# driskai/scenario_gym

Hardware: AMD Instinct MI355X
Metric: entity-steps/sec (batched rollout) (higher is better)
Workload: dtype f64

## Files before the change

scenario_gym_amd/csrc/h_queue.hip:

```cpp
#include "sgym_host.hpp"

using namespace sgh;

enum { Q_HOST_RING = 16 };
int sgh::check_queue(sg_handle *h)
{
    for (; h->q_count > 0; --h->q_count) {
        const unsigned *w = h->q_host + (size_t)((h->q_head - h->q_count + Q_HOST_RING) % Q_HOST_RING) * sg::Q_STATE_WORDS;
        const unsigned code = w[sg::Q_ERR];
        if (code == 0 || h->q_failed) continue;
        static const char *what[] = {"", "a rollout wavefront waited for the controller pre-pass", "a rollout wavefront waited for the previous chunk of its block",
                                     "the controller pre-pass waited for a buffer of the table ring"};
        h->q_failed = true;
        h->queue_mode = 0;
        snprintf(h->q_msg, sizeof h->q_msg, "sg_rollout: the persistent table launch gave up (%s longer than SG_QUEUE_TIMEOUT_MS; %u work items had finished): "
                                            "the state of the batch is undefined -- sg_reset / sg_upload before the next call", what[code < 4 ? code : 0],
                 w[sg::Q_ITEMS_DONE]);
    }
    return h->q_failed ? fail(h, SG_ERR_HIP, "%s", h->q_msg) : SG_OK;
}
void sgh::forget_queue_failure(sg_handle *h)
{
    h->q_count = 0;
    h->q_failed = false;
}

#define SG_QUEUE_FALLBACK 1
static size_t slots_of(sg_handle *h, bool rss)
{
    const size_t by_bounds = (size_t)h->n_simd * (size_t)(rss ? SG_WAVES_PER_SIMD : (h->planar ? SG_PLANAR_WAVES : SG_TAB_WAVES));
    if (h->q_waves_G != h->G) {
        std::fill(h->q_waves_per_cu, h->q_waves_per_cu + 3, -1);
        h->q_waves_G = h->G;
    }
    int &cached = h->q_waves_per_cu[rss ? 2 : (h->planar ? 1 : 0)];
    if (cached < 0) cached = rss ? sgl::rss_tabq_waves_per_cu(h->G) : sgl::tabq_waves_per_cu(h->G, h->planar);
    return cached > 0 ? std::min(by_bounds, (size_t)cached * (size_t)(h->n_simd / 4)) : by_bounds;
}
static int launch_queue(sg_handle *h, int n_steps, int force, const double *d_actions, int chunk, size_t *ev_next, bool rss = false)
{
    const size_t nblk = h->NE / 64, np = (size_t)h->p.n_ctl_pad, n_ctl_waves = np / 64;
    std::vector<int> len;
    chunk = std::min(chunk, std::max(1, env_int("SG_QUEUE_CAP", 512)));
    const int first = std::max(1, std::min(chunk, env_int("SG_QUEUE_FIRST", 160)));
    const int grow = std::max(101, env_int("SG_QUEUE_GROW", 140));
    const int decay = env_int("SG_QUEUE_DECAY", 140);
    std::vector<int> up, down;
    for (long long n = first; n < chunk && n < chunk * 3ll / 4; n = std::max(n + 1, n * grow / 100)) up.push_back((int)n);
    if (decay > 100)
        for (long long n = first; n < chunk && n < chunk * 3ll / 4; n = std::max(n + 1, n * decay / 100)) down.insert(down.begin(), (int)n);
    long long ramp = 0;
    for (int n : up) ramp += n;
    for (int n : down) ramp += n;
    if (ramp + chunk <= n_steps) {
        const long long mid = n_steps - ramp;
        const int whole = (int)(mid / chunk), rest = (int)(mid % chunk);
        len = up;
        len.insert(len.end(), (size_t)whole, chunk);
        if (rest > 0) down.insert(std::lower_bound(down.begin(), down.end(), rest, std::greater<int>()), rest);
        len.insert(len.end(), down.begin(), down.end());
    } else {
        for (int k0 = 0, n = 0; k0 < n_steps; k0 += n) {
            const long long want = len.empty() ? first : std::max<long long>((long long)len.back() + 1, (long long)len.back() * grow / 100);
            n = (int)std::min<long long>(std::min<long long>(chunk, want), n_steps - k0);
            if (want >= chunk / 2 + chunk / 4 && want < chunk) n = std::min(chunk, n_steps - k0);
            len.push_back(n);
        }
        while (len.size() > 1 && len.back() >= 2 * first && len.back() > 128) {
            const int L = len.back(), half = L / 2;
            len.back() = L - half;
            len.push_back(half);
        }
    }
    const int C = (int)len.size();
    if (C > sg::Q_MAX_CHUNKS) return SG_QUEUE_FALLBACK;
    const size_t row = (size_t)sg::CT_PLANES * sg::CT_W * np;
    const int ts = chunk;
    const size_t buf_bytes = (size_t)(ts + 1) * row * sizeof(double);
    int n_buf = C;
    {
        size_t free_b = 0, total_b = 0;
        if (hipMemGetInfo(&free_b, &total_b) != hipSuccess) { (void)hipGetLastError(); free_b = (size_t)8 << 30; }
        const size_t budget = std::min<size_t>((free_b + h->qtab_bytes) / 4, (size_t)std::max(1, env_int("SG_QUEUE_TAB_MB", 32768)) << 20);
        n_buf = (int)std::min<size_t>((size_t)C, std::max<size_t>(3, budget / buf_bytes));
        if (const int forced = env_int("SG_QUEUE_RING", 0)) n_buf = std::min(C, std::max(2, forced));
    }
    const size_t need = (size_t)n_buf * buf_bytes;
    if (need > h->qtab_bytes) {
        HIP_TRY(h, hipStreamSynchronize(h->stream));
        if (h->d_qtab) HIP_TRY(h, hipFree(h->d_qtab));
        h->d_qtab = nullptr;
        h->qtab_bytes = 0;
        if (hipMalloc((void **)&h->d_qtab, need) != hipSuccess) {
            (void)hipGetLastError();
            h->d_qtab = nullptr;
            return SG_QUEUE_FALLBACK;
        }
        h->qtab_bytes = need;
        poison(h->stream, h->d_qtab, need);
    }
    h->p.tab_steps = ts;
    const bool q_trace = env_int("SG_QUEUE_DEBUG", 0) != 0;
    const size_t words = (size_t)sg::Q_PROG_STRIDE * (1 + n_ctl_waves) + nblk + (size_t)sg::Q_MAX_CHUNKS + 1 + (size_t)sg::Q_SEATS + (q_trace ? nblk : 0);
    if (words * sizeof(unsigned) > h->qwords.cap) {
        HIP_TRY(h, hipStreamSynchronize(h->stream));
        if (const int rcw = h->qwords.ensure(h, words * sizeof(unsigned))) return rcw;
    }
    unsigned *const d_qwords = h->qwords.as<unsigned>();
    if (!h->q_host) HIP_TRY(h, hipHostMalloc((void **)&h->q_host, (size_t)Q_HOST_RING * sg::Q_STATE_WORDS * sizeof(unsigned), hipHostMallocDefault));
    if (h->q_count == Q_HOST_RING) {
        HIP_TRY(h, hipStreamSynchronize(h->stream));
        const int rcq = check_queue(h);
        if (rcq) return rcq;
    }
    HIP_TRY(h, hipMemsetAsync(d_qwords, 0, words * sizeof(unsigned), h->stream));
    sg::TabQueue tq{};
    tq.state = d_qwords;
    static_assert(sg::Q_STATE_WORDS <= sg::Q_PROG_STRIDE, "the state words have the first line to themselves");
    tq.ctl_prog = tq.state + sg::Q_PROG_STRIDE;
    tq.blk_prog = tq.ctl_prog + (size_t)sg::Q_PROG_STRIDE * n_ctl_waves;
    tq.chunk_cnt = tq.blk_prog + nblk;
    tq.seats = tq.chunk_cnt + sg::Q_MAX_CHUNKS + 1;
    tq.trace = q_trace ? tq.seats + sg::Q_SEATS : nullptr;
    tq.defer_ticks = (long long)std::max(1, env_int("SG_QUEUE_DEFER_US", 30)) * 100ll;
    tq.tab = h->d_qtab;
    tq.buf_doubles = buf_bytes / sizeof(double);
    tq.actions = d_actions;
    tq.timeout_ticks = (long long)std::max(1, env_int("SG_QUEUE_TIMEOUT_MS", 20000)) * 100000ll;
    if (const int us = env_int("SG_QUEUE_TIMEOUT_US", 0)) tq.timeout_ticks = (long long)std::max(1, us) * 100ll;
    tq.handoff = env_int("SG_QUEUE_HANDOFF", 1) != 0;
    tq.lag_prio = env_int("SG_QUEUE_LAGPRIO", 2);
    tq.nap = std::max(1, std::min(64, env_int("SG_QUEUE_NAP", 4)));
    const char *times_path = getenv("SG_QUEUE_TIMES");
    static unsigned long long *d_times = nullptr;
    static size_t times_cap = 0;
    const size_t n_times = (size_t)C * nblk * 4 + n_ctl_waves * (size_t)C;
    if (times_path && *times_path) {
        if (n_times > times_cap) {
            if (d_times) HIP_TRY(h, hipFree(d_times));
            HIP_TRY(h, hipMalloc((void **)&d_times, n_times * 8));
            times_cap = n_times;
        }
        HIP_TRY(h, hipMemsetAsync(d_times, 0, n_times * 8, h->stream));
        tq.times = d_times;
    }
    tq.n_chunks = C;
    tq.n_buf = n_buf;
    tq.nblk = (int)nblk;
    tq.n_ctl_waves = (int)n_ctl_waves;
    tq.k0[0] = 0;
    for (int c = 0; c < C; ++c) tq.k0[c + 1] = tq.k0[c] + len[(size_t)c];
    const size_t slots = slots_of(h, rss);
    const unsigned grid = (unsigned)std::min(slots, n_ctl_waves + nblk);
    hipEvent_t e0 = nullptr, e1 = nullptr;
    int rc;
    if ((rc = get_event(h, *ev_next, &e0)) || (rc = get_event(h, *ev_next + 1, &e1))) return rc;
    static hipStream_t ws = nullptr;
    static unsigned *w = nullptr;
    if (q_trace && !ws) {
        HIP_TRY(h, hipStreamCreateWithFlags(&ws, hipStreamNonBlocking));
        HIP_TRY(h, hipHostMalloc((void **)&w, (sg::Q_STATE_WORDS + 16) * sizeof(unsigned), hipHostMallocDefault));
        HIP_TRY(h, hipMemcpyAsync(w, d_qwords, 64, hipMemcpyDeviceToHost, ws));
        HIP_TRY(h, hipStreamSynchronize(ws));
    }
    HIP_TRY(h, hipEventRecord(e0, h->stream));
    note_queue(h, rss);
    if (rss) sgl::rollout_rss_tabq(h->G, dim3(grid), h->stream, h->p, h->cfg.timestep, force, tq);
    else sgl::rollout_tabq(h->G, h->planar, dim3(grid), h->stream, h->p, h->cfg.timestep, force, tq);
    HIP_TRY(h, hipGetLastError());
    HIP_TRY(h, hipEventRecord(e1, h->stream));
    HIP_TRY(h, hipMemcpyAsync(h->q_host + (size_t)h->q_head * sg::Q_STATE_WORDS, d_qwords, sg::Q_STATE_WORDS * sizeof(unsigned), hipMemcpyDeviceToHost, h->stream));
    h->q_head = (h->q_head + 1) % Q_HOST_RING;
    ++h->q_count;
    if (tq.times) {
        std::vector<unsigned long long> ht(n_times + 4);
        HIP_TRY(h, hipMemcpyAsync(ht.data() + 4, d_times, n_times * 8, hipMemcpyDeviceToHost, h->stream));
        HIP_TRY(h, hipStreamSynchronize(h->stream));
        ht[0] = (unsigned long long)C; ht[1] = nblk; ht[2] = n_ctl_waves; ht[3] = grid;
        if (FILE *f = fopen(times_path, "wb")) {
            fwrite(ht.data(), 8, ht.size(), f);
            fwrite(tq.k0, sizeof(int), (size_t)C + 1, f);
            fclose(f);
        }
    }
    if (const int dbg = env_int("SG_QUEUE_DEBUG", 0)) {
        fprintf(stderr, "queue: grid %u, %d chunks, ring %d, %zu blocks, %zu pre-pass wavefronts, first chunk %d steps\n", grid, C, n_buf, nblk, n_ctl_waves, len[0]);
        const int us = std::max(50, env_int("SG_QUEUE_DEBUG_US", 100000));
        const auto t_start = std::chrono::steady_clock::now();
        for (int i = 0; i < dbg; ++i) {
            std::this_thread::sleep_for(std::chrono::microseconds(us));
            if (hipMemcpyAsync(w, d_qwords, sg::Q_STATE_WORDS * sizeof(unsigned), hipMemcpyDeviceToHost, ws) != hipSuccess ||
                hipMemcpy2DAsync(w + sg::Q_STATE_WORDS, sizeof(unsigned), tq.ctl_prog, sg::Q_PROG_STRIDE * sizeof(unsigned), sizeof(unsigned),
                                 std::min<size_t>(4, n_ctl_waves), hipMemcpyDeviceToHost, ws) != hipSuccess ||
                hipStreamSynchronize(ws) != hipSuccess) break;
            fprintf(stderr, "queue +%.2f ms: tickets %u head %u err %u items done %u | ctl_prog %u %u %u %u",
                    std::chrono::duration<double, std::milli>(std::chrono::steady_clock::now() - t_start).count(), w[0], w[1], w[2], w[3], w[8], w[9], w[10], w[11]);
            unsigned *tr = w + sg::Q_STATE_WORDS + 8;
            if (hipMemcpyAsync(tr, tq.trace, 8 * sizeof(unsigned), hipMemcpyDeviceToHost, ws) == hipSuccess && hipStreamSynchronize(ws) == hipSuccess)
                fprintf(stderr, " | trace (chunk << 8 | stage) of blocks 0..7: %x %x %x %x %x %x %x %x", tr[0], tr[1], tr[2], tr[3], tr[4], tr[5], tr[6], tr[7]);
            fprintf(stderr, "\n");
            if (hipStreamQuery(h->stream) == hipSuccess) break;
        }
// ... 110 lines not shown
```

scenario_gym_amd/csrc/sgym_control.hpp:

```cpp
#pragma once

namespace sg {

struct CtlLds { double ctrl[9][64]; double seg[5][64]; };

template <bool FAST, bool RIDERS = false>
__device__ __forceinline__ void control_body_l(CtlLds &lds ,
                                               const unsigned qblock ,
                                               const Params &p, double timestep, int n_steps, int first, int k0,
                                               const double *actions , double *tab, int row0, int metrics)
{
    const int lane = threadIdx.x;
    const size_t q = (size_t)qblock * 64 + lane;
    const int ent_raw = p.ctl_ent[q];
    const bool active = ent_raw >= 0;
    const uint32_t ent = active ? (uint32_t)ent_raw : 0u;
    const uint32_t r = ent / (uint32_t)p.EP;
    const LanePtr st(p.stat + (size_t)(ent >> 6) * (ST_COUNT * 64), (ent & 63) * 8u);
    const LanePtr dy(p.dyn + (size_t)(ent >> 6) * ((size_t)p.FROWS * 64), (ent & 63) * 8u);
    const int64_t meta = fld<int64_t>(st, ST_META);
    const int kind = active ? (int)(meta & 0xff) : SG_KIND_NONE;
    const double min_t = fld(st, ST_MIN_T), bl = fld(st, ST_BL);
    const bool is_ego = active && (int)(ent - r * (uint32_t)p.EP) == p.sstat[r].ego;
#pragma unroll
    for (int c = 0; c < 9; ++c) lds.ctrl[c][lane] = fld(st, ST_CTRL + c);
    const size_t NP = (size_t)p.n_ctl_pad;
    double *cst = p.ctl_state + q;

    double pose[6], t, prev_t;
    double m_avg, m_max, m_t;
    bool present;
    CtrlState cs;
    if (first) {
        const sg_scenario_state &sd = p.sdyn[r];
        t = sd.t;
        prev_t = sd.prev_t;
        m_avg = sd.ego_avg_speed; m_max = sd.ego_max_speed; m_t = sd.avg_t;
        present = fld<uint64_t>(dy, SG_F_PRESENT) != 0;
#pragma unroll
        for (int c = 0; c < 6; ++c) pose[c] = fld(dy, SG_F_POSE + c);
        cs.speed = fld(dy, SG_F_CTRL + 0); cs.e_lon_prev = fld(dy, SG_F_CTRL + 1);
        cs.e_lat_prev = fld(dy, SG_F_CTRL + 2); cs.e_lon_int = fld(dy, SG_F_CTRL + 3);
    } else {
#pragma unroll
        for (int c = 0; c < 6; ++c) pose[c] = cst[(CS_POSE + c) * NP];
        present = cst[CS_PRESENT * NP] != 0.0;
        cs.speed = cst[(CS_CTRL + 0) * NP]; cs.e_lon_prev = cst[(CS_CTRL + 1) * NP];
        cs.e_lat_prev = cst[(CS_CTRL + 2) * NP]; cs.e_lon_int = cst[(CS_CTRL + 3) * NP];
        t = cst[CS_T * NP];
        prev_t = cst[CS_PREV_T * NP];
        m_avg = cst[(CS_METRIC + 0) * NP]; m_max = cst[(CS_METRIC + 1) * NP]; m_t = cst[(CS_METRIC + 2) * NP];
    }
    if (!active) present = false;

    Table T;
    {
        const double *kn = p.knots + fld<int64_t>(st, ST_KNOT_OFF) * 7;
        T.x = kn; T.xs = 7; T.y = kn + 1; T.ys = 7; T.cs = 1;
        T.n = active ? (int)(meta >> 32) : 0;
    }
    double seg_hi;
    int seg_cur;
    double sgr[5] = {0.0, 0.0, 0.0, 0.0, 0.0};
    auto seg_publish = [&](const Segment &S) {
        lds.seg[0][lane] = S.x_lo;
// ... 28 lines not shown
    const RecipDiv rd_l(active ? bl : 1.0), rd_10(10.0);
    double cpr[9];
#pragma unroll
    for (int c = 0; c < 9; ++c) cpr[c] = FAST ? fld(st, ST_CTRL + c) : 0.0;
    sg_loads_done();

    for (int k = 0; k < n_steps; ++k) {
        const double *Kp = SG_TRIG;
        if (!FAST) asm volatile("" : "+s"(Kp));
        ConstTbl K = (ConstTbl)Kp;
        const double next_t = t + timestep;
        const double state_dt = t - prev_t;
        const double dt = next_t - t;
        if (FAST && fast_kind && sg_all(!active || (present && !(next_t > seg_hi) && __builtin_fabs(pose[3]) < 1.0e5))) {
            const double dq = next_t - sgr[0];
            const double tx = sgr[3] * dq + sgr[1], ty = sgr[4] * dq + sgr[2];
            double sin_h, cos_h;
            sg_sincos_core(pose[3], sin_h, cos_h, K);
            const double e0 = tx - pose[0], e1 = ty - pose[1];
            const double e_lon = cos_h * e0 + sin_h * e1;
            const double e_lat = -sin_h * e0 + cos_h * e1;
            const double speed0 = cs.speed;
            const double g_mid = 1.0 - rd_10.div(0.9 * (speed0 - 5.0));
            const double gain = (speed0 > 5.0 && speed0 <= 15) ? g_mid : (speed0 > 15 ? 0.1 : 1.0);
            const RecipDiv rd(state_dt);
            const double d_lat = e_lat - cs.e_lat_prev, d_lon = e_lon - cs.e_lon_prev;
            const double e_lat_D = rd.div(d_lat);
            const double kp = cpr[SG_C_STEER_KP] * gain, kd = cpr[SG_C_STEER_KD] * gain;
            double steer = kp * e_lat + kd * e_lat_D;
            const double e_lon_D = rd.div(d_lon);
            const double e_lon_I = cs.e_lon_int + e_lon * state_dt;
            double accel = cpr[SG_C_ACCEL_KP] * e_lon + cpr[SG_C_ACCEL_KD] * e_lon_D + cpr[SG_C_ACCEL_KI] * e_lon_I;
            accel = __builtin_fabs(e_lon) > 0.1 ? accel : 0.0;
            const double max_steer = cpr[SG_C_MAX_STEER], max_accel = cpr[SG_C_MAX_ACCEL];
            const double max_speed = cpr[SG_C_MAX_SPEED], allow_rev = cpr[SG_C_ALLOW_REVERSE];
            accel = __builtin_fmin(__builtin_fmax(accel, -max_accel), max_accel);
            steer = __builtin_fmin(__builtin_fmax(steer, -max_steer), max_steer);
            const double dxs = speed0 * cos_h, dys = speed0 * sin_h;
            double tan_s = sg_tan_poly(steer, K);
            const bool steep = !(__builtin_fabs(steer) < 0.67434);
            if (sg_any(steep & active)) {
                double s2, c2;
                sg_sincos_core(steer, s2, c2, K);
                tan_s = steep ? s2 / c2 : tan_s;
            }
            const double hnum = speed0 * tan_s;
            const double dh = hnum == 0.0 ? hnum : rd_l.div(hnum);
            const double nx = pose[0] + dxs * dt, ny = pose[1] + dys * dt, nh = pose[3] + dh * dt;
            double nspeed = speed0 + accel * dt;
            nspeed = allow_rev == 0.0 ? __builtin_fmax(0.0, nspeed) : nspeed;
            nspeed = max_speed == max_speed ? __builtin_fmin(max_speed, nspeed) : nspeed;
            bool ok = rd.safe(d_lat) & rd.safe(d_lon) & (__builtin_fabs(steer) < 1.0e5) & (rd_l.safe(hnum) | (hnum == 0.0));
            double n_avg = m_avg, n_max = m_max, n_mt = m_t;
            if (metrics) {
                const RecipDiv rdt(dt), rnt(next_t);
                const double ax = nx - pose[0], ay = ny - pose[1];
                const double az = pose[2] - pose[2];
                const double speed = sg_norm3(rdt.div(ax), rdt.div(ay), 0.0);
                const double w = rnt.div(m_t);
                n_avg = m_avg + (1.0 - w) * (speed - m_avg);
                n_max = __builtin_fmax(speed, m_max);
                n_mt = next_t;
                ok = ok & (!is_ego | (rdt.safe(ax) & rdt.safe(ay) & rnt.safe(m_t) & (dt > 0.0) & (az == 0.0)));
            }
            if (sg_all(!active || ok)) {
                cs.e_lat_prev = e_lat; cs.e_lon_prev = e_lon; cs.e_lon_int = e_lon_I; cs.speed = nspeed;
                pose[0] = nx; pose[1] = ny; pose[3] = nh;
                if (is_ego) { m_avg = n_avg; m_max = n_max; m_t = n_mt; }
                prev_t = t;
                t = next_t;
                *reinterpret_cast<double4 *>(out + (size_t)k * CT_W) = make_double4(pose[0], pose[1], pose[3], cs.speed);
                *reinterpret_cast<double4 *>(out1 + (size_t)k * CT_W) = make_double4(cs.e_lon_prev, cs.e_lat_prev, cs.e_lon_int, 0.0);
                if (is_ego && metrics) *reinterpret_cast<double4 *>(out2 + (size_t)k * CT_W) = make_double4(m_avg, m_max, m_t, 0.0);
                continue;
            }
        }
        double act_a = 0.0, act_s = 0.0;
        if (kind == SG_KIND_AGENT_VEHICLE && actions) {
            const double *a = actions + ((size_t)(k0 + k) * p.R + r) * 2;
            act_a = a[0];
            act_s = a[1];
        }
        if (next_t > seg_hi) {
            Segment S;
            S.x_hi = seg_hi;
            S.cur = seg_cur;
            seg_advance(T, S, next_t);
            seg_publish(S);
            sg_loads_done();
        }
        double np_[6];
        const double dq = next_t - lds.seg[0][lane];
        np_[0] = lds.seg[3][lane] * dq + lds.seg[1][lane];
        np_[1] = lds.seg[4][lane] * dq + lds.seg[2][lane];
        bool npres = false;
        if (RIDERS && replay_lane) {
            if (next_t > SR.x_hi) { seg_advance(TR, SR, next_t); sg_loads_done(); }
            const double dqr = next_t - SR.x_lo;
#pragma unroll
            for (int c = 0; c < 6; ++c) np_[c] = SR.sl[c] * dqr + SR.ylo[c];
            npres = kind == SG_KIND_REPLAY ? (p.persist || is_static || (next_t >= min_t && next_t <= max_t))
                                           : (present || min_t >= t);
        } else if (present) {
            npres = true;
            const double tx = np_[0], ty = np_[1];
#pragma unroll
            for (int c = 0; c < 6; ++c) np_[c] = pose[c];
            double sin_h, cos_h;
            sg_sincos(pose[3], sin_h, cos_h, K);
            auto cp = [&](int q) -> double { return lds.ctrl[q][lane]; };
            if (kind == SG_KIND_AGENT_PID)
                pid_step(cs, cp, bl, state_dt, dt, tx, ty, sin_h, cos_h, np_, K);
            else
                vehicle_step(cs, cp, bl, dt, act_a, act_s, sin_h, cos_h, np_, K);
        } else if (active && min_t >= t) {
            npres = true;
            Segment S;
            S.cur = seg_cur;
            seg_load(T, S);
            sg_loads_done();
            const double dqs = next_t - S.x_lo;
#pragma unroll
            for (int c = 0; c < 6; ++c) np_[c] = S.sl[c] * dqs + S.ylo[c];
        }
        if (is_ego && npres && metrics) {
            double prev[6];
            if (!present) {
                own_position_extrap(T.x, T.n, t, prev);
                sg_loads_done();
            } else {
#pragma unroll
                for (int c = 0; c < 6; ++c) prev[c] = pose[c];
            }
            const double v0 = (np_[0] - prev[0]) / dt, v1 = (np_[1] - prev[1]) / dt, v2 = (np_[2] - prev[2]) / dt;
            const double speed = sg_norm3(v0, v1, v2);
            const double w = m_t / next_t;
            m_avg += (1.0 - w) * (speed - m_avg);
            m_t = next_t;
            m_max = __builtin_fmax(speed, m_max);
        }
        present = npres;
        if (npres) {
#pragma unroll
            for (int c = 0; c < 6; ++c) pose[c] = np_[c];
        }
        prev_t = t;
        t = next_t;
        *reinterpret_cast<double4 *>(out + (size_t)k * CT_W) = make_double4(pose[0], pose[1], pose[3], cs.speed);
        *reinterpret_cast<double4 *>(out1 + (size_t)k * CT_W) = make_double4(cs.e_lon_prev, cs.e_lat_prev, cs.e_lon_int, 0.0);
        if (is_ego && metrics) *reinterpret_cast<double4 *>(out2 + (size_t)k * CT_W) = make_double4(m_avg, m_max, m_t, 0.0);
        if (RIDERS) *reinterpret_cast<double4 *>(out2 + (size_t)k * CT_W) = make_double4(pose[2], pose[4], pose[5], present ? 1.0 : 0.0);
    }
#pragma unroll
    for (int c = 0; c < 6; ++c) cst[(CS_POSE + c) * NP] = pose[c];
    cst[CS_PRESENT * NP] = present ? 1.0 : 0.0;
    cst[(CS_CTRL + 0) * NP] = cs.speed; cst[(CS_CTRL + 1) * NP] = cs.e_lon_prev;
    cst[(CS_CTRL + 2) * NP] = cs.e_lat_prev; cst[(CS_CTRL + 3) * NP] = cs.e_lon_int;
    cst[CS_T * NP] = t;
    cst[CS_PREV_T * NP] = prev_t;
    cst[(CS_METRIC + 0) * NP] = m_avg; cst[(CS_METRIC + 1) * NP] = m_max; cst[(CS_METRIC + 2) * NP] = m_t;
}

template <bool FAST, bool RIDERS = false>
__device__ __forceinline__ void control_body(const Params &p, double timestep, int n_steps, int first, int k0,
                                             const double *actions , double *tab, int row0, int metrics)
{
    __shared__ CtlLds lds;
    control_body_l<FAST, RIDERS>(lds, blockIdx.x, p, timestep, n_steps, first, k0, actions, tab, row0, metrics);
}

#ifdef SG_UNIT_CTL
static __global__ __launch_bounds__(64, SG_CTL_WAVES) void control_kernel(Params p, double timestep, int n_steps, int first, int k0,
                                                     const double *actions , double *tab, int row0, int metrics)
{
    control_body<false>(p, timestep, n_steps, first, k0, actions, tab, row0, metrics);
}
#endif
#ifdef SG_UNIT_CTL
static __global__ __launch_bounds__(64, 2) void control_kernel_riders(Params p, double timestep, int n_steps, int first, int k0,
                                                               const double *actions , double *tab, int row0, int metrics)
{
    control_body<false, true>(p, timestep, n_steps, first, k0, actions, tab, row0, 0);
}
#endif
#ifdef SG_UNIT_CTL
static __global__ __launch_bounds__(64, 1) void control_kernel_fast(Params p, double timestep, int n_steps, int first, int k0,
                                                             const double *actions , double *tab, int row0, int metrics)
{
#ifdef SG_CTL_SETPRIO
    __builtin_amdgcn_s_setprio(3);
#endif
    control_body<true>(p, timestep, n_steps, first, k0, actions, tab, row0, metrics);
}
#endif

}
```

scenario_gym_amd/csrc/sgym_core.hpp:

```cpp
#pragma once

namespace sg {

enum {
    ST_BW = 0, ST_BL, ST_BCX, ST_BCY,
    ST_MIN_T, ST_MAX_T,
    ST_KNOT_OFF,
    ST_META,
    ST_ROUTE,
    ST_CTL,
    ST_CTRL,
    NCTRL_ROWS = 13,
    ST_COUNT = ST_CTRL + NCTRL_ROWS
};
constexpr uint32_t ROW = 512;

struct ScenStatic {
    double t0, length;
    int64_t grid_off;
    int32_t grid_n, ego;
};

struct RoadNet { double x0, y0, inv_cell; int32_t nx, ny; int64_t cell_base; };
struct RoadCand { int32_t poly; uint32_t edge_off; uint16_t n_edges; uint8_t ref_sel, ref_inside; };
// ... 17 lines not shown
struct Params {
    int R, E, EP;
    int persist;
    unsigned term_mask;
    int rec_cap, ev_cap;
    const double *stat;
    const ScenStatic *sstat;
    const double *knots;
    const double *grid_t;
    double *grid_y;
    double *dyn;
    sg_scenario_state *sdyn;
    sg_event *events;
    double *ev_pose;
    double *ev_hpose;
    double *rec_t, *rec_pose;
    const double *routes;
    const double *gon;
    int WV, FROWS;
    sg_social_force sf;
    const int32_t *ctl_ent;
    double *ctl_state;
    int n_ctl_pad;
    const double *ext_pose;
    int32_t *rss_state, *rss_code, *rss_seen;
    double *rss_safe;
    double *rssq;
    int32_t *rssq_n;
    int32_t rssq_cap;
    const unsigned char *reset_mask;
    const RoadIndex *road;
    int ctl_general;
    int ped_serial;
    int quiet;
    int tab_steps;
    int noise_mode;
    double noise_std_lon, noise_std_lat;
    const double *noise_normals;
    long long noise_len;
    unsigned long long noise_seed;
    int ped_behaviour;
    int n_ped_models;
    const double *ped_models;
    const int32_t *model_of;
#ifdef SG_PHASE_TIMERS
    unsigned long long *phase_cycles;
#endif
};

enum { PM_BEHAVIOUR = 0, PM_SF = 1, PM_STD_LON = 13, PM_STD_LAT = 14, PM_W = 16 };
static_assert(sizeof(sg_social_force) == 12 * sizeof(double), "sg_social_force is twelve doubles");

enum { CT_X = 0, CT_Y, CT_H, CT_SPEED, CT_W = 4, CT_ELON = 0, CT_ELAT, CT_EINT, CT_MAVG = 0, CT_MMAX, CT_MT, CT_PLANES = 3 };
enum { CS_POSE = 0, CS_PRESENT = 6, CS_CTRL = 7, CS_T = 11, CS_PREV_T = 12, CS_METRIC = 13, CS_COUNT = 16 };

#define SG_GLOBAL __attribute__((address_space(1)))
struct LanePtr {
    SG_GLOBAL char *a[3];
    __device__ __forceinline__ LanePtr(const double *blk, uint32_t voff)
    {
        a[0] = (SG_GLOBAL char *)(reinterpret_cast<char *>(const_cast<double *>(blk)) + voff);
        a[1] = a[0] + 8 * ROW;
        a[2] = a[0] + 16 * ROW;
        asm("" : "+v"(a[1]), "+v"(a[2]));
    }
};
template <typename T = double>
__device__ __forceinline__ T fld(const LanePtr &lp, int f)
{
    const int b = f < 24 ? f >> 3 : 2;
    return *reinterpret_cast<SG_GLOBAL const T *>(lp.a[b] + (f - 8 * b) * (int)ROW);
}
template <typename T>
__device__ __forceinline__ void stf(const LanePtr &lp, int f, T v)
{
    const int b = f < 24 ? f >> 3 : 2;
    *reinterpret_cast<SG_GLOBAL T *>(lp.a[b] + (f - 8 * b) * (int)ROW) = v;
}

__device__ __forceinline__ double sg_norm3(double a, double b, double c)
{
    return __builtin_sqrt(__builtin_fma(c, c, __builtin_fma(b, b, a * a)));
}
__device__ __forceinline__ double sg_norm2(double a, double b)
{
    return __builtin_sqrt(__builtin_fma(b, b, a * a));
}

__device__ __noinline__ double2 sg_sincos_slow(double x)
{
    return make_double2(sin(x), cos(x));
}

static __constant__ double SG_TRIG[48] = {
    6.36619772367581382433e-01,
    1.57079632673412561417e+00,
    6.07710050630396597660e-11,
    2.02226624879595063154e-21,
    -1.66666666666666324348e-01, 8.33333333332248946124e-03, -1.98412698298579493134e-04,
    2.75573137070700676789e-06, -2.50507602534068634195e-08, 1.58969099521155010221e-10,
    4.16666666666666019037e-02, -1.38888888888741095749e-03, 2.48015872894767294178e-05,
    -2.75573143513906633035e-07, 2.08757232129817482790e-09, -1.13596475577881948265e-11,
    3.33333333333334091986e-01, 1.33333333333201242699e-01, 5.39682539762260521377e-02,
    2.18694882948595424599e-02, 8.86323982359930005737e-03, 3.59207910759131235356e-03,
    1.45620945432529025516e-03, 5.88041240820264096874e-04, 2.46463134818469906812e-04,
    7.81794442939557092300e-05, 7.14072491382608190305e-05, -1.85586374855275456654e-05,
    2.59073051863633712884e-05, 0.0, 0.0, 0.0,
// ... 306 lines not shown
```

scenario_gym_amd/csrc/sgym_queue.hpp:

```cpp
#pragma once

namespace sg {

enum { Q_TICKET = 0, Q_HEAD = 1, Q_ERR = 2, Q_ITEMS_DONE = 3, Q_CTL_CLAIMED = 4, Q_STATE_WORDS = 8 };
constexpr int Q_SEATS = 1 << 14;
enum { Q_ERR_CTL_WAIT = 1, Q_ERR_BLOCK_WAIT = 2, Q_ERR_RING_WAIT = 3 };
constexpr int Q_MAX_CHUNKS = 255;
constexpr int Q_PROG_STRIDE = 32;

struct TabQueue {
    unsigned *state;
    unsigned *ctl_prog;
    unsigned *blk_prog;
    unsigned *chunk_cnt;
    unsigned *seats;
    long long defer_ticks;
    double *tab;
    size_t buf_doubles;
    const double *actions;
    unsigned *trace;
    unsigned long long *times;
    long long timeout_ticks;
    int n_chunks, n_buf, nblk, n_ctl_waves;
    int nap;
    int lag_prio;
    int handoff;
    int k0[Q_MAX_CHUNKS + 1];
};

__device__ __forceinline__ unsigned q_peek(const unsigned *w)
{
    return (unsigned)__builtin_amdgcn_readfirstlane((int)__hip_atomic_load(w, __ATOMIC_RELAXED, __HIP_MEMORY_SCOPE_AGENT));
}

__device__ __forceinline__ bool q_wait_ge(const unsigned *w, unsigned want, const TabQueue &tq, unsigned code)
{
    if (q_peek(w) >= want) return true;
    const long long t0 = wall_clock64();
    for (int spin = 0;; ++spin) {
        if (spin < 4) __builtin_amdgcn_s_sleep(16);
        else if (spin < 12) __builtin_amdgcn_s_sleep(112);
        else {
            const int n = min(tq.nap, 1 << min((spin - 12) >> 2, 6));
            for (int i = 0; i < n; ++i) __builtin_amdgcn_s_sleep(127);
        }
        if (q_peek(w) >= want) return true;
        if ((spin & 7) == 7 && q_peek(tq.state + Q_ERR) != 0) return false;
        if (wall_clock64() - t0 > tq.timeout_ticks) {
            if (threadIdx.x == 0) atomicCAS(tq.state + Q_ERR, 0u, code);
            return false;
        }
    }
}

__device__ __forceinline__ void q_acquire()
{
    __builtin_amdgcn_fence(__ATOMIC_ACQUIRE, "agent");
    asm volatile("s_dcache_inv\n\ts_waitcnt lgkmcnt(0)" ::: "memory");
}

__device__ __forceinline__ void q_release()
{
    asm volatile("s_waitcnt vmcnt(0)" ::: "memory");
    __builtin_amdgcn_fence(__ATOMIC_RELEASE, "agent");
    asm volatile("s_waitcnt vmcnt(0)" ::: "memory");
}

template <int G>
__device__ __forceinline__ void q_handoff_writethrough(const Params &p, unsigned b, int lane)
{
    asm volatile("s_waitcnt vmcnt(0)" ::: "memory");
    typedef SG_GLOBAL unsigned long long gu64;
    constexpr int FR = SG_F_COLL + 1;
    gu64 *rows = (gu64 *)(p.dyn + (size_t)b * ((size_t)FR * 64)) + lane;
    unsigned long long v[FR];
#pragma unroll
    for (int f = 0; f < FR; ++f) v[f] = __hip_atomic_load(rows + f * 64, __ATOMIC_RELAXED, __HIP_MEMORY_SCOPE_AGENT);
#pragma unroll
    for (int f = 0; f < FR; ++f) __hip_atomic_store(rows + f * 64, v[f], __ATOMIC_RELAXED, __HIP_MEMORY_SCOPE_AGENT);
    static_assert(sizeof(sg_scenario_state) % 8 == 0, "scenario records are copied in 8-byte words");
    constexpr int SW = (int)(sizeof(sg_scenario_state) / 8);
    const int gl = (int)b * 64 + lane, r = gl / G, slot = gl & (G - 1);
    if (r < p.R) {
        gu64 *sd = (gu64 *)(p.sdyn + r);
        for (int w = slot; w < SW; w += G) {
            const unsigned long long v = __hip_atomic_load(sd + w, __ATOMIC_RELAXED, __HIP_MEMORY_SCOPE_AGENT);
            __hip_atomic_store(sd + w, v, __ATOMIC_RELAXED, __HIP_MEMORY_SCOPE_AGENT);
        }
    }
    asm volatile("s_waitcnt vmcnt(0)" ::: "memory");
}

template <int G, unsigned F>
__device__ __forceinline__ void tabq_body(const Params &p, double timestep, int force, const TabQueue &tq)
{
    constexpr bool RSS = (F & V_RSS) != 0;
    using Tile = typename Variant<G, 1, F>::Lds;
    static_assert(sizeof(Tile) >= sizeof(CtlLds), "the pre-pass role lays its LDS over the tile");
    __shared__ Tile lds;
    __shared__ typename std::conditional<RSS, RssQueue, char>::type rssq_lds;
    const int lane = threadIdx.x;
    unsigned ticket = ~0u;
    {
        const unsigned hw = (unsigned)__builtin_amdgcn_s_getreg((4 << 0) | (0 << 6) | (31 << 11));
        const unsigned xcc = (unsigned)__builtin_amdgcn_s_getreg((20 << 0) | (0 << 6) | (3 << 11));
        const unsigned seat = ((xcc & 15u) << 10) | (((hw >> 13) & 7u) << 7) | (((hw >> 12) & 1u) << 6) | (((hw >> 8) & 15u) << 2) | ((hw >> 4) & 3u);
        unsigned rank = 0;
        if (lane == 0) {
            atomicAdd(tq.state + Q_TICKET, 1u);
            rank = atomicAdd(tq.seats + seat, 1u);
        }
        rank = (unsigned)__builtin_amdgcn_readfirstlane((int)rank);
        bool claim = rank == 0 && q_peek(tq.state + Q_CTL_CLAIMED) < (unsigned)tq.n_ctl_waves;
        if (rank != 0) {
            const long long t0 = wall_clock64();
            while (q_peek(tq.state + Q_CTL_CLAIMED) < (unsigned)tq.n_ctl_waves) {
                if (wall_clock64() - t0 > tq.defer_ticks) { claim = true; break; }
                __builtin_amdgcn_s_sleep(8);
            }
        }
        if (claim) {
            unsigned idx = 0;
            if (lane == 0) idx = atomicAdd(tq.state + Q_CTL_CLAIMED, 1u);
            idx = (unsigned)__builtin_amdgcn_readfirstlane((int)idx);
            if (idx < (unsigned)tq.n_ctl_waves) ticket = idx;
        }
    }

    if (ticket < (unsigned)tq.n_ctl_waves) {
        __builtin_amdgcn_s_setprio(3);
        CtlLds &cl = *reinterpret_cast<CtlLds *>(&lds);
        for (int c = 0; c < tq.n_chunks; ++c) {
            if (c >= tq.n_buf && !q_wait_ge(tq.chunk_cnt + (c - tq.n_buf), (unsigned)tq.nblk, tq, Q_ERR_RING_WAIT)) break;
            control_body_l<true>(cl, ticket, p, timestep, tq.k0[c + 1] - tq.k0[c], c == 0, tq.k0[c], tq.actions,
                                 tq.tab + (size_t)(c % tq.n_buf) * tq.buf_doubles, 0, RSS ? 0 : 1);
            q_release();
            if (tq.times && lane == 0) tq.times[(size_t)tq.n_chunks * tq.nblk * 4 + (size_t)ticket * tq.n_chunks + c] = wall_clock64();
            if (lane == 0) __hip_atomic_store(tq.ctl_prog + ticket * Q_PROG_STRIDE, (unsigned)(c + 1), __ATOMIC_RELAXED, __HIP_MEMORY_SCOPE_AGENT);
        }
        __builtin_amdgcn_s_setprio(0);
        if (q_peek(tq.state + Q_ERR) != 0) return;
    }

    const unsigned n_items = (unsigned)tq.n_chunks * (unsigned)tq.nblk;
    unsigned done_b = ~0u, done_c = 0;
    for (;;) {
        unsigned item = 0;
        if (lane == 0) {
            if (done_b != ~0u) {
                __hip_atomic_store(tq.blk_prog + done_b, done_c + 1, __ATOMIC_RELAXED, __HIP_MEMORY_SCOPE_AGENT);
                if (tq.n_buf < tq.n_chunks) atomicAdd(tq.chunk_cnt + done_c, 1u);
                atomicAdd(tq.state + Q_ITEMS_DONE, 1u);
            }
            item = atomicAdd(tq.state + Q_HEAD, 1u);
        }
        item = (unsigned)__builtin_amdgcn_readfirstlane((int)item);
        done_b = ~0u;
        if (item >= n_items) break;
        const unsigned c = item / (unsigned)tq.nblk, b = item - c * (unsigned)tq.nblk;
        auto trace = [&](unsigned stage) {
            if (tq.trace && lane == 0) __hip_atomic_store(tq.trace + b, (c << 8) | stage, __ATOMIC_RELAXED, __HIP_MEMORY_SCOPE_AGENT);
        };
        trace(1);
        auto stamp = [&](int k) {
            if (tq.times && lane == 0) tq.times[(size_t)item * 4 + k] = wall_clock64();
        };
        stamp(0);
        if (tq.lag_prio) __builtin_amdgcn_s_setprio(0);
        const bool behind = c != 0 && q_peek(tq.blk_prog + b) < c;
        bool ok = c == 0 || q_wait_ge(tq.blk_prog + b, c, tq, Q_ERR_BLOCK_WAIT);
        {
            const LanePtr st(p.stat + (size_t)b * (ST_COUNT * 64), (uint32_t)lane * 8u);
            const int64_t cq = fld<int64_t>(st, ST_CTL);
            uint64_t m = __ballot(cq >= 0);
            while (m && ok) {
                const int l = __builtin_ctzll(m);
                m &= m - 1;
                const unsigned w = (unsigned)__builtin_amdgcn_readlane((int)(uint32_t)cq, l) >> 6;
                ok = q_wait_ge(tq.ctl_prog + w * Q_PROG_STRIDE, c + 1, tq, Q_ERR_CTL_WAIT);
            }
        }
        if (!ok) break;
        if (tq.lag_prio && behind) {
            if (tq.lag_prio == 1) __builtin_amdgcn_s_setprio(1);
            else __builtin_amdgcn_s_setprio(2);
        }
        trace(2);
        q_acquire();
        trace(3);
        stamp(1);
        const double *tab = tq.tab + (size_t)(c % (unsigned)tq.n_buf) * tq.buf_doubles;
        const int gl = (int)b * 64 + lane, r_raw = gl / G;
        const bool in_range = r_raw < p.R;
        const int r = in_range ? r_raw : p.R - 1;
        const int ev_before = p.ev_cap > 0 ? min(p.sdyn[r].n_events, p.ev_cap) : 0;
        rollout_body_l<G, 1, F>(lds, p, timestep, tq.k0[c + 1] - tq.k0[c], 0, force, nullptr, tab, SliceArgs{}, b);
        trace(4);
        stamp(2);
        if (RSS) {
            asm volatile("s_waitcnt vmcnt(0)" ::: "memory");
            rss_lines_block(p, (RssQueueLds)&rssq_lds, (size_t)b);
        }
        if (!RSS && p.ev_cap > 0) {
            asm volatile("s_waitcnt vmcnt(0)" ::: "memory");
            const int ev_after = in_range ? min(p.sdyn[r].n_events, p.ev_cap) : 0;
            if (ev_after > ev_before) {
                int64_t ectl;
                const bool from_tab = ego_table_column(p, r, ectl);
                for (int i = ev_before + (gl & (G - 1)); i < ev_after; i += G) event_take_table_pose(p, r, i, tab, from_tab, ectl);
            }
        }
        trace(5);
        if (RSS) {
            asm volatile("s_waitcnt vmcnt(0)" ::: "memory");
            typedef SG_GLOBAL int gi32;
            typedef SG_GLOBAL unsigned long long gu64;
            const size_t idx = (size_t)b * 64 + lane;
            gi32 *sw = (gi32 *)(p.rss_state + idx), *cw = (gi32 *)(p.rss_code + idx);
            gu64 *fw = (gu64 *)(p.rss_safe + idx * 2);
            const int v0 = __hip_atomic_load(sw, __ATOMIC_RELAXED, __HIP_MEMORY_SCOPE_AGENT);
            const int v1 = __hip_atomic_load(cw, __ATOMIC_RELAXED, __HIP_MEMORY_SCOPE_AGENT);
            const unsigned long long v2 = __hip_atomic_load(fw, __ATOMIC_RELAXED, __HIP_MEMORY_SCOPE_AGENT);
            const unsigned long long v3 = __hip_atomic_load(fw + 1, __ATOMIC_RELAXED, __HIP_MEMORY_SCOPE_AGENT);
            __hip_atomic_store(sw, v0, __ATOMIC_RELAXED, __HIP_MEMORY_SCOPE_AGENT);
            __hip_atomic_store(cw, v1, __ATOMIC_RELAXED, __HIP_MEMORY_SCOPE_AGENT);
            __hip_atomic_store(fw, v2, __ATOMIC_RELAXED, __HIP_MEMORY_SCOPE_AGENT);
            __hip_atomic_store(fw + 1, v3, __ATOMIC_RELAXED, __HIP_MEMORY_SCOPE_AGENT);
            const int glr = (int)b * 64 + lane;
            if ((glr & (G - 1)) == 0 && glr / G < p.R) {
                gi32 *nw = (gi32 *)(p.rss_seen + glr / G);
                const int v4 = __hip_atomic_load(nw, __ATOMIC_RELAXED, __HIP_MEMORY_SCOPE_AGENT);
                __hip_atomic_store(nw, v4, __ATOMIC_RELAXED, __HIP_MEMORY_SCOPE_AGENT);
            }
        }
        if (tq.handoff == 1) q_handoff_writethrough<G>(p, b, lane);
        else q_release();
        trace(6);
        stamp(3);
        done_b = b;
        done_c = c;
    }
    if (lane == 0 && done_b != ~0u) {
        __hip_atomic_store(tq.blk_prog + done_b, done_c + 1, __ATOMIC_RELAXED, __HIP_MEMORY_SCOPE_AGENT);
        if (tq.n_buf < tq.n_chunks) atomicAdd(tq.chunk_cnt + done_c, 1u);
        atomicAdd(tq.state + Q_ITEMS_DONE, 1u);
    }
}

template <int G>
__global__ __launch_bounds__(64, SG_TAB_WAVES) __attribute__((amdgpu_num_vgpr(SG_TAB_VGPR))) void rollout_kernel_tabq(
    Params p, double timestep, int force, TabQueue tq)
{
    tabq_body<G, V_TAB | V_HAST>(p, timestep, force, tq);
}
template <int G>
__global__ __launch_bounds__(64, SG_PLANAR_WAVES) __attribute__((amdgpu_num_vgpr(SG_PLANAR_VGPR))) void rollout_kernel_tabq_planar(
    Params p, double timestep, int force, TabQueue tq)
{
    tabq_body<G, V_TAB | V_HAST | V_PLANAR>(p, timestep, force, tq);
}

template <int G>
__global__ __launch_bounds__(64, SG_WAVES_PER_SIMD) void rollout_kernel_rss_tabq(Params p, double timestep, int force, TabQueue tq)
{
    tabq_body<G, V_RSS | V_CTAB>(p, timestep, force, tq);
}

}
```

Measured before the change: 149.9 billion.

## Defer ego metric accumulation from controller pre-pass to separate queue work items

The controller pre-pass stops computing the running ego speed average and maximum inline. It now writes a per-step speed tag into the table, and new per-controller-wave metric work items in the persistent queue scan each chunk to accumulate the metrics. Rollout blocks wait on the metric progress counters before copying the final metrics into scenario state. The aim is to shorten the serial controller critical path. In exchange the queue gains extra items, extra waits and more progress words, and ring reuse now also depends on the metric items finishing.

```diff
diff --git a/scenario_gym_amd/csrc/h_queue.hip b/scenario_gym_amd/csrc/h_queue.hip
--- a/scenario_gym_amd/csrc/h_queue.hip
+++ b/scenario_gym_amd/csrc/h_queue.hip
@@ -10,11 +10,12 @@
         const unsigned code = w[sg::Q_ERR];
         if (code == 0 || h->q_failed) continue;
         static const char *what[] = {"", "a rollout wavefront waited for the controller pre-pass", "a rollout wavefront waited for the previous chunk of its block",
-                                     "the controller pre-pass waited for a buffer of the table ring"};
+                                     "the controller pre-pass waited for a buffer of the table ring",
+                                     "a wavefront waited for the ego metrics of a chunk"};
         h->q_failed = true;
         h->queue_mode = 0;
         snprintf(h->q_msg, sizeof h->q_msg, "sg_rollout: the persistent table launch gave up (%s longer than SG_QUEUE_TIMEOUT_MS; %u work items had finished): "
-                                            "the state of the batch is undefined -- sg_reset / sg_upload before the next call", what[code < 4 ? code : 0],
+                                            "the state of the batch is undefined -- sg_reset / sg_upload before the next call", what[code < 5 ? code : 0],
                  w[sg::Q_ITEMS_DONE]);
     }
     return h->q_failed ? fail(h, SG_ERR_HIP, "%s", h->q_msg) : SG_OK;
@@ -101,7 +102,9 @@
     }
     h->p.tab_steps = ts;
     const bool q_trace = env_int("SG_QUEUE_DEBUG", 0) != 0;
-    const size_t words = (size_t)sg::Q_PROG_STRIDE * (1 + n_ctl_waves) + nblk + (size_t)sg::Q_MAX_CHUNKS + 1 + (size_t)sg::Q_SEATS + (q_trace ? nblk : 0);
+    const char *met_env = getenv("SG_QUEUE_METRICS");
+    const size_t n_met = rss || (met_env && !strcmp(met_env, "inline")) ? 0 : n_ctl_waves;
+    const size_t words = (size_t)sg::Q_PROG_STRIDE * (1 + 2 * n_ctl_waves) + nblk + (size_t)sg::Q_MAX_CHUNKS + 1 + (size_t)sg::Q_SEATS + (q_trace ? nblk : 0);
     if (words * sizeof(unsigned) > h->qwords.cap) {
         HIP_TRY(h, hipStreamSynchronize(h->stream));
         if (const int rcw = h->qwords.ensure(h, words * sizeof(unsigned))) return rcw;
@@ -118,7 +121,8 @@
     tq.state = d_qwords;
     static_assert(sg::Q_STATE_WORDS <= sg::Q_PROG_STRIDE, "the state words have the first line to themselves");
     tq.ctl_prog = tq.state + sg::Q_PROG_STRIDE;
-    tq.blk_prog = tq.ctl_prog + (size_t)sg::Q_PROG_STRIDE * n_ctl_waves;
+    tq.met_prog = tq.ctl_prog + (size_t)sg::Q_PROG_STRIDE * n_ctl_waves;
+    tq.blk_prog = tq.met_prog + (size_t)sg::Q_PROG_STRIDE * n_ctl_waves;
     tq.chunk_cnt = tq.blk_prog + nblk;
     tq.seats = tq.chunk_cnt + sg::Q_MAX_CHUNKS + 1;
     tq.trace = q_trace ? tq.seats + sg::Q_SEATS : nullptr;
@@ -134,7 +138,7 @@
     const char *times_path = getenv("SG_QUEUE_TIMES");
     static unsigned long long *d_times = nullptr;
     static size_t times_cap = 0;
-    const size_t n_times = (size_t)C * nblk * 4 + n_ctl_waves * (size_t)C;
+    const size_t n_times = (size_t)C * nblk * 4 + n_ctl_waves * (size_t)C + 2 * n_met * (size_t)C;
     if (times_path && *times_path) {
         if (n_times > times_cap) {
             if (d_times) HIP_TRY(h, hipFree(d_times));
@@ -148,6 +152,7 @@
     tq.n_buf = n_buf;
     tq.nblk = (int)nblk;
     tq.n_ctl_waves = (int)n_ctl_waves;
+    tq.n_met = (int)n_met;
     tq.k0[0] = 0;
     for (int c = 0; c < C; ++c) tq.k0[c + 1] = tq.k0[c] + len[(size_t)c];
     const size_t slots = slots_of(h, rss);
diff --git a/scenario_gym_amd/csrc/sgym_control.hpp b/scenario_gym_amd/csrc/sgym_control.hpp
--- a/scenario_gym_amd/csrc/sgym_control.hpp
+++ b/scenario_gym_amd/csrc/sgym_control.hpp
@@ -4,13 +4,14 @@
 
 struct CtlLds { double ctrl[9][64]; double seg[5][64]; };
 
-template <bool FAST, bool RIDERS = false>
+template <bool FAST, bool RIDERS = false, bool DEFER = false>
 __device__ __forceinline__ void control_body_l(CtlLds &lds ,
                                                const unsigned qblock ,
                                                const Params &p, double timestep, int n_steps, int first, int k0,
                                                const double *actions , double *tab, int row0, int metrics)
 {
     const int lane = threadIdx.x;
+    const bool deferred = DEFER && metrics == CTL_METRICS_DEFERRED;
     const size_t q = (size_t)qblock * 64 + lane;
     const int ent_raw = p.ctl_ent[q];
     const bool active = ent_raw >= 0;
@@ -145,7 +146,9 @@
             nspeed = max_speed == max_speed ? __builtin_fmin(max_speed, nspeed) : nspeed;
             bool ok = rd.safe(d_lat) & rd.safe(d_lon) & (__builtin_fabs(steer) < 1.0e5) & (rd_l.safe(hnum) | (hnum == 0.0));
             double n_avg = m_avg, n_max = m_max, n_mt = m_t;
-            if (metrics) {
+            if (deferred) {
+                ok = ok & (!is_ego | (pose[2] - pose[2] == 0.0));
+            } else if (metrics) {
                 const RecipDiv rdt(dt), rnt(next_t);
                 const double ax = nx - pose[0], ay = ny - pose[1];
                 const double az = pose[2] - pose[2];
@@ -163,8 +166,9 @@
                 prev_t = t;
                 t = next_t;
                 *reinterpret_cast<double4 *>(out + (size_t)k * CT_W) = make_double4(pose[0], pose[1], pose[3], cs.speed);
-                *reinterpret_cast<double4 *>(out1 + (size_t)k * CT_W) = make_double4(cs.e_lon_prev, cs.e_lat_prev, cs.e_lon_int, 0.0);
-                if (is_ego && metrics) *reinterpret_cast<double4 *>(out2 + (size_t)k * CT_W) = make_double4(m_avg, m_max, m_t, 0.0);
+                *reinterpret_cast<double4 *>(out1 + (size_t)k * CT_W) =
+                    make_double4(cs.e_lon_prev, cs.e_lat_prev, cs.e_lon_int, deferred ? CT_SPD_DERIVE : 0.0);
+                if (is_ego && metrics && !deferred) *reinterpret_cast<double4 *>(out2 + (size_t)k * CT_W) = make_double4(m_avg, m_max, m_t, 0.0);
                 continue;
             }
         }
@@ -216,6 +220,7 @@
 #pragma unroll
             for (int c = 0; c < 6; ++c) np_[c] = S.sl[c] * dqs + S.ylo[c];
         }
+        double spd_tag = deferred ? CT_SPD_NONE : 0.0;
         if (is_ego && npres && metrics) {
             double prev[6];
             if (!present) {
@@ -227,10 +232,13 @@
             }
             const double v0 = (np_[0] - prev[0]) / dt, v1 = (np_[1] - prev[1]) / dt, v2 = (np_[2] - prev[2]) / dt;
             const double speed = sg_norm3(v0, v1, v2);
-            const double w = m_t / next_t;
-            m_avg += (1.0 - w) * (speed - m_avg);
-            m_t = next_t;
-            m_max = __builtin_fmax(speed, m_max);
+            if (deferred) spd_tag = speed;
+            else {
+                const double w = m_t / next_t;
+                m_avg += (1.0 - w) * (speed - m_avg);
+                m_t = next_t;
+                m_max = __builtin_fmax(speed, m_max);
+            }
         }
         present = npres;
         if (npres) {
@@ -240,8 +248,8 @@
         prev_t = t;
         t = next_t;
         *reinterpret_cast<double4 *>(out + (size_t)k * CT_W) = make_double4(pose[0], pose[1], pose[3], cs.speed);
-        *reinterpret_cast<double4 *>(out1 + (size_t)k * CT_W) = make_double4(cs.e_lon_prev, cs.e_lat_prev, cs.e_lon_int, 0.0);
-        if (is_ego && metrics) *reinterpret_cast<double4 *>(out2 + (size_t)k * CT_W) = make_double4(m_avg, m_max, m_t, 0.0);
+        *reinterpret_cast<double4 *>(out1 + (size_t)k * CT_W) = make_double4(cs.e_lon_prev, cs.e_lat_prev, cs.e_lon_int, spd_tag);
+        if (is_ego && metrics && !deferred) *reinterpret_cast<double4 *>(out2 + (size_t)k * CT_W) = make_double4(m_avg, m_max, m_t, 0.0);
         if (RIDERS) *reinterpret_cast<double4 *>(out2 + (size_t)k * CT_W) = make_double4(pose[2], pose[4], pose[5], present ? 1.0 : 0.0);
     }
 #pragma unroll
@@ -251,7 +259,9 @@
     cst[(CS_CTRL + 2) * NP] = cs.e_lat_prev; cst[(CS_CTRL + 3) * NP] = cs.e_lon_int;
     cst[CS_T * NP] = t;
     cst[CS_PREV_T * NP] = prev_t;
-    cst[(CS_METRIC + 0) * NP] = m_avg; cst[(CS_METRIC + 1) * NP] = m_max; cst[(CS_METRIC + 2) * NP] = m_t;
+    if (!deferred) {
+        cst[(CS_METRIC + 0) * NP] = m_avg; cst[(CS_METRIC + 1) * NP] = m_max; cst[(CS_METRIC + 2) * NP] = m_t;
+    }
 }
 
 template <bool FAST, bool RIDERS = false>
diff --git a/scenario_gym_amd/csrc/sgym_core.hpp b/scenario_gym_amd/csrc/sgym_core.hpp
--- a/scenario_gym_amd/csrc/sgym_core.hpp
+++ b/scenario_gym_amd/csrc/sgym_core.hpp
@@ -93,7 +93,11 @@
 static_assert(sizeof(sg_social_force) == 12 * sizeof(double), "sg_social_force is twelve doubles");
 
 enum { CT_X = 0, CT_Y, CT_H, CT_SPEED, CT_W = 4, CT_ELON = 0, CT_ELAT, CT_EINT, CT_MAVG = 0, CT_MMAX, CT_MT, CT_PLANES = 3 };
-enum { CS_POSE = 0, CS_PRESENT = 6, CS_CTRL = 7, CS_T = 11, CS_PREV_T = 12, CS_METRIC = 13, CS_COUNT = 16 };
+enum { CT_SPD = 3 };
+constexpr double CT_SPD_DERIVE = -1.0;
+constexpr double CT_SPD_NONE = -2.0;
+enum { CTL_METRICS_DEFERRED = 2 };
+enum { CS_POSE = 0, CS_PRESENT = 6, CS_CTRL = 7, CS_T = 11, CS_PREV_T = 12, CS_METRIC = 13, CS_MET_T = 16, CS_MET_X = 17, CS_MET_Y = 18, CS_COUNT = 19 };
 
 #define SG_GLOBAL __attribute__((address_space(1)))
 struct LanePtr {
diff --git a/scenario_gym_amd/csrc/sgym_queue.hpp b/scenario_gym_amd/csrc/sgym_queue.hpp
--- a/scenario_gym_amd/csrc/sgym_queue.hpp
+++ b/scenario_gym_amd/csrc/sgym_queue.hpp
@@ -4,13 +4,14 @@
 
 enum { Q_TICKET = 0, Q_HEAD = 1, Q_ERR = 2, Q_ITEMS_DONE = 3, Q_CTL_CLAIMED = 4, Q_STATE_WORDS = 8 };
 constexpr int Q_SEATS = 1 << 14;
-enum { Q_ERR_CTL_WAIT = 1, Q_ERR_BLOCK_WAIT = 2, Q_ERR_RING_WAIT = 3 };
+enum { Q_ERR_CTL_WAIT = 1, Q_ERR_BLOCK_WAIT = 2, Q_ERR_RING_WAIT = 3, Q_ERR_MET_WAIT = 4 };
 constexpr int Q_MAX_CHUNKS = 255;
 constexpr int Q_PROG_STRIDE = 32;
 
 struct TabQueue {
     unsigned *state;
     unsigned *ctl_prog;
+    unsigned *met_prog;
     unsigned *blk_prog;
     unsigned *chunk_cnt;
     unsigned *seats;
@@ -22,6 +23,7 @@
     unsigned long long *times;
     long long timeout_ticks;
     int n_chunks, n_buf, nblk, n_ctl_waves;
+    int n_met;
     int nap;
     int lag_prio;
     int handoff;
@@ -91,6 +93,62 @@
     asm volatile("s_waitcnt vmcnt(0)" ::: "memory");
 }
 
+__device__ __forceinline__ void q_metric_item(const Params &p, double timestep, const TabQueue &tq, unsigned w, unsigned c, double *tab)
+{
+    const int lane = threadIdx.x;
+    const size_t q = (size_t)w * 64 + lane;
+    const int ent_raw = p.ctl_ent[q];
+    const bool active = ent_raw >= 0;
+    const uint32_t ent = active ? (uint32_t)ent_raw : 0u;
+    const uint32_t r = ent / (uint32_t)p.EP;
+    const bool is_ego = active && (int)(ent - r * (uint32_t)p.EP) == p.sstat[r].ego;
+    const size_t NP = (size_t)p.n_ctl_pad;
+    double *cst = p.ctl_state + q;
+    double t = 0.0, m_avg = 0.0, m_max = 0.0, m_t = 0.0, px = 0.0, py = 0.0;
+    if (is_ego) {
+        if (c == 0) {
+            const sg_scenario_state &sd = p.sdyn[r];
+            const LanePtr dy(p.dyn + (size_t)(ent >> 6) * ((size_t)p.FROWS * 64), (ent & 63) * 8u);
+            t = sd.t;
+            m_avg = sd.ego_avg_speed; m_max = sd.ego_max_speed; m_t = sd.avg_t;
+            px = fld(dy, SG_F_POSE + 0); py = fld(dy, SG_F_POSE + 1);
+        } else {
+            m_avg = cst[(CS_METRIC + 0) * NP]; m_max = cst[(CS_METRIC + 1) * NP]; m_t = cst[(CS_METRIC + 2) * NP];
+            t = cst[CS_MET_T * NP]; px = cst[CS_MET_X * NP]; py = cst[CS_MET_Y * NP];
+        }
+    }
+    const size_t plane = NP * ((size_t)(p.tab_steps + 1) * CT_W);
+    const double *in0 = tab + q * (size_t)(p.tab_steps + 1) * CT_W;
+    const double *in1 = in0 + plane;
+    double *out2 = tab + q * (size_t)(p.tab_steps + 1) * CT_W + 2 * plane;
+    const int n = tq.k0[c + 1] - tq.k0[c];
+    if (is_ego) {
+#pragma unroll 8
+        for (int k = 0; k < n; ++k) {
+            const double2 xy = *reinterpret_cast<const double2 *>(in0 + (size_t)k * CT_W);
+            const double tag = in1[(size_t)k * CT_W + CT_SPD];
+            const double next_t = t + timestep;
+            const double dt = next_t - t;
+            double speed = tag;
+            if (tag == CT_SPD_DERIVE) {
+                const double v0 = (xy.x - px) / dt, v1 = (xy.y - py) / dt, v2 = 0.0 / dt;
+                speed = sg_norm3(v0, v1, v2);
+            }
+            if (tag != CT_SPD_NONE) {
+                const double wt = m_t / next_t;
+                m_avg += (1.0 - wt) * (speed - m_avg);
+                m_t = next_t;
+                m_max = __builtin_fmax(speed, m_max);
+            }
+            px = xy.x; py = xy.y;
+            t = next_t;
+            *reinterpret_cast<double4 *>(out2 + (size_t)k * CT_W) = make_double4(m_avg, m_max, m_t, 0.0);
+        }
+        cst[(CS_METRIC + 0) * NP] = m_avg; cst[(CS_METRIC + 1) * NP] = m_max; cst[(CS_METRIC + 2) * NP] = m_t;
+        cst[CS_MET_T * NP] = t; cst[CS_MET_X * NP] = px; cst[CS_MET_Y * NP] = py;
+    }
+}
+
 template <int G, unsigned F>
 __device__ __forceinline__ void tabq_body(const Params &p, double timestep, int force, const TabQueue &tq)
 {
@@ -131,9 +189,9 @@
         __builtin_amdgcn_s_setprio(3);
         CtlLds &cl = *reinterpret_cast<CtlLds *>(&lds);
         for (int c = 0; c < tq.n_chunks; ++c) {
-            if (c >= tq.n_buf && !q_wait_ge(tq.chunk_cnt + (c - tq.n_buf), (unsigned)tq.nblk, tq, Q_ERR_RING_WAIT)) break;
-            control_body_l<true>(cl, ticket, p, timestep, tq.k0[c + 1] - tq.k0[c], c == 0, tq.k0[c], tq.actions,
-                                 tq.tab + (size_t)(c % tq.n_buf) * tq.buf_doubles, 0, RSS ? 0 : 1);
+            if (c >= tq.n_buf && !q_wait_ge(tq.chunk_cnt + (c - tq.n_buf), (unsigned)(tq.nblk + tq.n_met), tq, Q_ERR_RING_WAIT)) break;
+            control_body_l<true, false, !RSS>(cl, ticket, p, timestep, tq.k0[c + 1] - tq.k0[c], c == 0, tq.k0[c], tq.actions,
+                                 tq.tab + (size_t)(c % tq.n_buf) * tq.buf_doubles, 0, RSS ? 0 : (tq.n_met ? (int)CTL_METRICS_DEFERRED : 1));
             q_release();
             if (tq.times && lane == 0) tq.times[(size_t)tq.n_chunks * tq.nblk * 4 + (size_t)ticket * tq.n_chunks + c] = wall_clock64();
             if (lane == 0) __hip_atomic_store(tq.ctl_prog + ticket * Q_PROG_STRIDE, (unsigned)(c + 1), __ATOMIC_RELAXED, __HIP_MEMORY_SCOPE_AGENT);
@@ -142,13 +200,15 @@
         if (q_peek(tq.state + Q_ERR) != 0) return;
     }
 
-    const unsigned n_items = (unsigned)tq.n_chunks * (unsigned)tq.nblk;
+    const unsigned n_met = RSS ? 0u : (unsigned)tq.n_met, per_chunk = n_met + (unsigned)tq.nblk;
+    const unsigned n_items = (unsigned)tq.n_chunks * per_chunk + n_met;
     unsigned done_b = ~0u, done_c = 0;
     for (;;) {
         unsigned item = 0;
         if (lane == 0) {
             if (done_b != ~0u) {
-                __hip_atomic_store(tq.blk_prog + done_b, done_c + 1, __ATOMIC_RELAXED, __HIP_MEMORY_SCOPE_AGENT);
+                unsigned *prog = done_b < (unsigned)tq.nblk ? tq.blk_prog + done_b : tq.met_prog + (done_b - (unsigned)tq.nblk) * Q_PROG_STRIDE;
+                __hip_atomic_store(prog, done_c + 1, __ATOMIC_RELAXED, __HIP_MEMORY_SCOPE_AGENT);
                 if (tq.n_buf < tq.n_chunks) atomicAdd(tq.chunk_cnt + done_c, 1u);
                 atomicAdd(tq.state + Q_ITEMS_DONE, 1u);
             }
@@ -157,13 +217,33 @@
         item = (unsigned)__builtin_amdgcn_readfirstlane((int)item);
         done_b = ~0u;
         if (item >= n_items) break;
-        const unsigned c = item / (unsigned)tq.nblk, b = item - c * (unsigned)tq.nblk;
+        const unsigned c_blk = item < n_met ? 0u : (item - n_met) / per_chunk, j = item < n_met ? item : item - n_met - c_blk * per_chunk;
+        if (!RSS && j < n_met) {
+            const unsigned c = item < n_met ? 0u : c_blk + 1;
+            if (c >= (unsigned)tq.n_chunks) continue;
+            if (tq.lag_prio) __builtin_amdgcn_s_setprio(0);
+            if (!q_wait_ge(tq.ctl_prog + j * Q_PROG_STRIDE, c + 1, tq, Q_ERR_CTL_WAIT)) break;
+            if (c != 0 && !q_wait_ge(tq.met_prog + j * Q_PROG_STRIDE, c, tq, Q_ERR_MET_WAIT)) break;
+            __builtin_amdgcn_s_setprio(2);
+            q_acquire();
+            const size_t ts = (size_t)tq.n_chunks * tq.nblk * 4 + (size_t)tq.n_ctl_waves * tq.n_chunks + ((size_t)j * tq.n_chunks + c) * 2;
+            if (tq.times && lane == 0) tq.times[ts] = wall_clock64();
+            q_metric_item(p, timestep, tq, j, c, tq.tab + (size_t)(c % (unsigned)tq.n_buf) * tq.buf_doubles);
+            q_release();
+            __builtin_amdgcn_s_setprio(0);
+            if (tq.times && lane == 0) tq.times[ts + 1] = wall_clock64();
+            done_b = (unsigned)tq.nblk + j;
+            done_c = c;
+            continue;
+        }
+        const unsigned c = c_blk, b = j - n_met;
+        const unsigned ritem = c * (unsigned)tq.nblk + b;
         auto trace = [&](unsigned stage) {
             if (tq.trace && lane == 0) __hip_atomic_store(tq.trace + b, (c << 8) | stage, __ATOMIC_RELAXED, __HIP_MEMORY_SCOPE_AGENT);
         };
         trace(1);
         auto stamp = [&](int k) {
-            if (tq.times && lane == 0) tq.times[(size_t)item * 4 + k] = wall_clock64();
+            if (tq.times && lane == 0) tq.times[(size_t)ritem * 4 + k] = wall_clock64();
         };
         stamp(0);
         if (tq.lag_prio) __builtin_amdgcn_s_setprio(0);
@@ -194,6 +274,7 @@
         const bool in_range = r_raw < p.R;
         const int r = in_range ? r_raw : p.R - 1;
         const int ev_before = p.ev_cap > 0 ? min(p.sdyn[r].n_events, p.ev_cap) : 0;
+        const int steps_before = p.sdyn[r].n_steps;
         rollout_body_l<G, 1, F>(lds, p, timestep, tq.k0[c + 1] - tq.k0[c], 0, force, nullptr, tab, SliceArgs{}, b);
         trace(4);
         stamp(2);
@@ -208,6 +289,32 @@
                 int64_t ectl;
                 const bool from_tab = ego_table_column(p, r, ectl);
                 for (int i = ev_before + (gl & (G - 1)); i < ev_after; i += G) event_take_table_pose(p, r, i, tab, from_tab, ectl);
+            }
+        }
+        if (!RSS && n_met) {
+            asm volatile("s_waitcnt vmcnt(0)" ::: "memory");
+            int64_t mctl = -1;
+            int last = -1;
+            if (in_range && (gl & (G - 1)) == 0) {
+                const int n_done = __hip_atomic_load(&p.sdyn[r].n_steps, __ATOMIC_RELAXED, __HIP_MEMORY_SCOPE_AGENT) - steps_before;
+                if (n_done > 0 && ego_table_column(p, r, mctl)) last = n_done - 1;
+            }
+            const uint64_t need = __ballot(last >= 0);
+            for (uint64_t m = need; m && ok;) {
+                const int l = __builtin_ctzll(m);
+                m &= m - 1;
+                const unsigned w = (unsigned)__builtin_amdgcn_readlane((int)(uint32_t)mctl, l) >> 6;
+                ok = q_wait_ge(tq.met_prog + w * Q_PROG_STRIDE, c + 1, tq, Q_ERR_MET_WAIT);
+            }
+            if (!ok) break;
+            if (need) {
+                q_acquire();
+                if (last >= 0) {
+                    const size_t lane_stride = (size_t)(p.tab_steps + 1) * CT_W;
+                    const double *lr2 = tab + (size_t)mctl * lane_stride + (size_t)last * CT_W + 2 * (size_t)p.n_ctl_pad * lane_stride;
+                    sg_scenario_state &sx = p.sdyn[r];
+                    sx.ego_avg_speed = lr2[CT_MAVG]; sx.ego_max_speed = lr2[CT_MMAX]; sx.avg_t = lr2[CT_MT];
+                }
             }
         }
         trace(5);
@@ -241,7 +348,8 @@
         done_c = c;
     }
     if (lane == 0 && done_b != ~0u) {
-        __hip_atomic_store(tq.blk_prog + done_b, done_c + 1, __ATOMIC_RELAXED, __HIP_MEMORY_SCOPE_AGENT);
+        unsigned *prog = done_b < (unsigned)tq.nblk ? tq.blk_prog + done_b : tq.met_prog + (done_b - (unsigned)tq.nblk) * Q_PROG_STRIDE;
+        __hip_atomic_store(prog, done_c + 1, __ATOMIC_RELAXED, __HIP_MEMORY_SCOPE_AGENT);
         if (tq.n_buf < tq.n_chunks) atomicAdd(tq.chunk_cnt + done_c, 1u);
         atomicAdd(tq.state + Q_ITEMS_DONE, 1u);
     }
```

New measurement: 146.3 billion. 2.4% lower.
